# johnomotani/SharedMemSparseLU.jl

Measured on AMD Instinct MI355X. Metric: nnz(L+U)/s + achieved HBM GB/s, 3D Poisson 128³ numeric LU, 1/2/4/8 GPU, higher is better.
Workload: dtype f64

## Files before the change

sharedmemsparselu.jl_amd/csrc/plan.hpp:

```cpp
#pragma once
#include <algorithm>
#include <cstdint>
#include <string>
#include <vector>

namespace smlu {

struct Tune {
  int ob = 0;
  int64_t t128_min = 512;
  bool small_k = true;
  int64_t fullpiv_ns = -1;
  int64_t f22_gather_nu = 512;
  int64_t f22_gather_ch = 8;
  int64_t lside_min = 2048;
  int sweep_spin = 1 << 22;
  bool solve_steps = false;
  bool no_graph = false;
  bool debug_sync = false;
  bool no_repivot = false;
  int host_threads = 0;
};
Tune tune();


struct PlanOptions {
  int ordering = 0;
  int64_t grid[3] = {0, 0, 0};
  int relax = 1;
  int64_t leaf_size = 64;
  std::vector<int64_t> preorder;
};

struct Graph {
  int64_t n = 0;
  std::vector<int64_t> ptr;
  std::vector<int32_t> adj;
};

Graph build_sym_graph(int64_t n, const int64_t* colptr, const int32_t* rowval);
std::vector<int64_t> order_geometric_nd(int64_t nx, int64_t ny, int64_t nz, int64_t leaf);
std::vector<int64_t> order_graph_nd(const Graph& g, int64_t leaf);
std::vector<int64_t> order_amd(const Graph& g);
std::vector<int64_t> compute_order(int64_t n, const int64_t* colptr, const int32_t* rowval,
                                   const PlanOptions& opt, std::string& err);
std::vector<int64_t> zero_free_diagonal(int64_t n, const int64_t* colptr, const int32_t* rowval,
                                        const double* a);

struct Plan {
  int64_t n = 0, nnzA = 0;
  std::vector<int64_t> Acolptr;
  std::vector<int32_t> Arow;
  bool sym_pattern = false;

  std::vector<int64_t> q, qinv;
  std::vector<int64_t> p0, p0inv;
  bool given_order = false;
  bool matched = false;
  int perm_parity = 0;
  int pair_parity = -1;

  int64_t ntsup = 0;
  std::vector<int64_t> t_first;
  std::vector<int64_t> t_rowptr;
  std::vector<int32_t> t_rows;
  std::vector<int32_t> col2t;

  int64_t nsup = 0;
  std::vector<int64_t> s_first;
  std::vector<int64_t> s_parent;
  std::vector<int64_t> s_rowptr;
  std::vector<int32_t> s_rows;
  std::vector<int32_t> col2s;
  std::vector<int32_t> s_level;
  std::vector<int64_t> ch_ptr;
  std::vector<int32_t> ch_list;
  std::vector<int32_t> child_rank;
  std::vector<int32_t> relmap;
  int nlevels = 0;
  std::vector<int64_t> lev_ptr;
  std::vector<int32_t> lev_sup;

  std::vector<int64_t> Loff, Uoff;
  std::vector<int64_t> lev_foff;
  int64_t factor_size = 0;
  std::vector<int64_t> Foff;
  std::vector<int64_t> lev_soff, lev_ssize;
  int64_t scratch_size = 0;

  std::vector<int64_t> Adest;
  std::vector<int32_t> A_s, A_li, A_lj;
  std::vector<int64_t> Alev_ptr;
  std::vector<int32_t> Alev_ent;
  std::vector<int64_t> Arowptr;
  std::vector<int32_t> Arow_ent;

  double nnzL = 0, nnzU = 0;
  double upd = 0;
  double flops = 0;
  double stored = 0;
  int64_t front_max = 0, ns_max = 0, nu_max = 0;
  double analysis_ms = 0;
  double phase_ms[12] = {0};

  int nparts = 1;
  int64_t dob = 384;
// ... 51 lines not shown
```

sharedmemsparselu.jl_amd/csrc/schedule.hpp:

```cpp
#pragma once
#include <algorithm>
#include <cstdint>
#include <string>
#include <vector>

#include "device.hpp"
#include "plan.hpp"

namespace smlu {

constexpr int kSmallM = 128;
constexpr int kFullPivNs = 512;
constexpr int kNbFull = 32;
constexpr int kNbTile = 64;
constexpr int kSwapStride = 1 + 2 * 64;
constexpr int kOBDefault = 384;

enum Kind : int {
  K_EXTADD, K_FRONT_LDS, K_PANEL, K_TRSMU, K_TRSML,
  K_GEMM, K_FWD, K_BWD, K_FWDG, K_TRIF, K_BWDU, K_TRIB, K_GEMM22, K_LASWP, K_STEPTRSM, K_GEMMU,
  K_GEMMO, K_TRIINV, K_BWDU12C, K_VCOPY, K_FWDT, K_BWDT, K_SWEEPF, K_SWEEPB, K_UROWS, K_FWDP, K_NKIND
};
inline const char* const kKindName[] = {"assemble", "small", "panel",
                                  "trsm", "trsm", "gemm", "solve", "solve", "solve", "solve",
// ... 24 lines not shown
  int64_t so;
  int db;
  int64_t dof;
  int64_t bytes;
};

struct CommOp {
  int type = 0;
  std::vector<int32_t> peer;
  std::vector<int> sbase, rbase;
  std::vector<int64_t> soff, roff, sbytes, rbytes;
  int32_t root = -1;
  std::vector<int32_t> grp;
  int bbase = 4;
  int64_t bytes = 0;
  std::vector<HSeg> pack, unpack;
  int64_t pack0 = 0, unpack0 = 0;
  int at(int32_t p) {
    for (size_t i = 0; i < peer.size(); ++i)
      if (peer[i] == p) return (int)i;
    peer.push_back(p);
    sbase.push_back(4);
    rbase.push_back(5);
    soff.push_back(0);
    roff.push_back(0);
    sbytes.push_back(0);
    rbytes.push_back(0);
    return (int)peer.size() - 1;
  }
};

struct Operand {
  int buf = -1;
  int64_t off = 0;
  Operand operator+(int64_t d) const { return Operand{buf, off + d}; }
};
struct GemmRec {
  Operand A, B, C;
  int32_t m, n, k;
  int32_t lda, ldb, ldc;
  int32_t tiles_m = 0;
  int32_t gsid = -1;
  int64_t tile0 = 0;
  int32_t front = -1;
};

struct ScheduleInput {
  const Plan* plan = nullptr;
  const RankLayout* lay = nullptr;
  Tune tn;
  int rank = 0, nranks = 1;
  bool dominant = false;
  int pivmode = 0;
  bool cpair = false;
  bool use_mfma = true;
  int ob = kOBDefault;
};

struct Schedule {
  std::vector<SNode> hsn;
  std::vector<int32_t> node_front;
  int64_t nnodes = 0;
  std::vector<Launch> fac, fwd, bwd;
  std::vector<Launch> fwdm, bwdm;
  std::vector<size_t> fac_seg, fwd_seg, bwd_seg;
  std::vector<size_t> fwdm_seg, bwdm_seg;
  std::vector<int> fac_comm, fwd_comm, bwd_comm;
  std::vector<CommOp> comm;
  std::vector<int32_t> ilist;
  std::vector<XContrib> xt;
  std::vector<AEnt> ae;
  std::vector<XCol> xc;
  std::vector<FrontTile> ft;
  std::vector<int32_t> gptr, gent;
  std::vector<GemmRec> gt;
  std::vector<SwapTask> st_tasks;
  std::vector<URowTask> ur_tasks;
  std::vector<F22Gather> g22;
  std::vector<F22Child> g22ch;
  std::vector<int32_t> g22inv;
  int64_t f22_gather_fronts = 0;
  double f22_gather_entries = 0;
  int64_t side_launches = 0, side_rows = 0;
  double gemm_flops = 0, gemm22_flops = 0;
  double gemm_bytes = 0;
  int64_t gemm_launches = 0, gemm128_launches = 0;
  int64_t nlaunch = 0;
  int64_t max_list = 1;
  int64_t ssync_n = 0, ntick = 0;
  int64_t voff = 0;
  bool uses_tinv = false;
  int ob = kOBDefault;
  int64_t t128_min = 512;
  bool small_k = true;
  bool trsm_gemm = true;
  int err_code = 0;
};
constexpr int kSchedErrArg = -1, kSchedErrAlloc = -3, kSchedErrState = -6;

std::string build_schedule(const ScheduleInput& in, Schedule& out);
void rank_layout_of(const Plan& P, int rank, int nranks, RankLayout& Y);
void schedule_digest(const Schedule& S, const double bytes[5], std::vector<uint64_t>& out);

}
```

sharedmemsparselu.jl_amd/csrc/schedule_build.cpp:

```cpp
#include "schedule.hpp"

#include <limits>
#include <unordered_map>
#include <utility>

namespace smlu {
namespace {

const Operand kStore{0, 0}, kScratch{1, 0}, kBlockBuf{6, 0}, kTinv{7, 0};

GemmRec gemm_task(Operand A, Operand B, Operand C, int64_t m, int64_t n, int64_t k, int64_t lda, int64_t ldb,
                  int64_t ldc, int32_t gsid = -1) {
  GemmRec g;
  g.A = A; g.B = B; g.C = C;
  g.m = (int32_t)m; g.n = (int32_t)n; g.k = (int32_t)k;
  g.lda = (int32_t)lda; g.ldb = (int32_t)ldb; g.ldc = (int32_t)ldc;
  g.gsid = gsid;
  return g;
}
void update(std::vector<GemmRec>& cand, double& fl, Operand A, Operand B, Operand C, int64_t m, int64_t n, int64_t k,
            int64_t lda, int64_t ldb, int64_t ldc) {
  if (m <= 0 || n <= 0 || k <= 0) return;
  cand.push_back(gemm_task(A, B, C, m, n, k, lda, ldb, ldc));
  fl += 2.0 * (double)m * (double)n * (double)k;
// ... 21 lines not shown
  std::unordered_map<int64_t, int32_t> blkmap;
  std::vector<int64_t> fr_ptr;
  std::vector<int32_t> fr_ent;
  std::vector<int64_t> LP;
  std::vector<int32_t> LS;
  std::vector<std::vector<int32_t>> dfront;
  std::vector<char> dlevel;
  int64_t dist_slots = 0;
  int64_t spf = 0;
  int fuse_mode = 0;
  bool fuse_panel = false, fuse_inv = false, fuse_urows = false;
  std::vector<int64_t> bidx;
  std::vector<int32_t> col_cnt, col_pos;
  std::vector<std::vector<Launch>> bwd_levels;
  std::vector<char> f22g;
  int cur_level = 0;
  std::vector<size_t> lvl_end;

  Builder(const ScheduleInput& i, Schedule& s)
      : in(i), P(*i.plan), Y(*i.lay), S(s), rank(i.rank), nranks(i.nranks) {}

  static Launch launch(int kind, int step, size_t off) {
    Launch L;
    L.kind = kind;
    L.step = step;
    L.off = (int64_t)off;
    return L;
  }
  void fail(int code, const char* msg) {
    S.err_code = code;
    err = msg;
  }
  void add_comm(std::vector<Launch>& seq, std::vector<size_t>& seg, std::vector<int>& cm, CommOp&& op) {
    seg.push_back(seq.size());
    cm.push_back((int)S.comm.size());
    S.comm.push_back(std::move(op));
  }
  int32_t child_col(int64_t c, int64_t jc, int64_t* src) const {
    const int64_t nuc = P.nu(c);
    if (!P.dist(c)) {
      if (src && P.owner[c] == rank) *src = Y.Foff[c] + jc * nuc;
      return P.owner[c];
    }
    const int64_t b = P.npblk(c) + jc / P.dob;
    const int32_t o = P.blk_owner(c, b);
    if (src && o == rank) {
      const RankLayout::Blk& B = Y.blocks[blkmap.at((int64_t)c * 1048576 + b)];
      *src = B.foff + (P.ns(c) + jc - B.c0) * nuc;
    }
    return o;
  }
  int32_t node_of(int64_t s, int64_t b) const { return blknode[blkmap.at(s * 1048576 + b)]; }
  int32_t holder(int64_t c) const { return P.dist(c) ? P.blk_owner(c, P.npblk(c) - 1) : P.owner[c]; }
  bool gform(int64_t s) const { return S.trsm_gemm && S.hsn[s].nb == kNbTile; }
  int64_t slot_of(int64_t s, int64_t u) const { return dist_slots + bidx[s] * spf + u; }
  struct Step {
    int64_t kb, w, ostart, oend, R, M, slot;
  };
  Step geom(int64_t s, int64_t t) const {
    const SNode& r = S.hsn[s];
    Step g;
    g.M = (int64_t)r.ns + r.nu;
    g.kb = t * r.nb;
    g.w = std::min<int64_t>(r.nb, r.ns - g.kb);
    g.ostart = (g.kb / S.ob) * S.ob;
    g.oend = std::min<int64_t>(r.ns, g.ostart + S.ob);
    g.R = r.mode == 1 ? r.ns - g.kb : g.w;
    g.slot = slot_of(s, t % (S.ob / r.nb));
    return g;
  }
  void add_gemm_launch(std::vector<GemmRec>& cand, double fl, int step, int kind = K_GEMM, bool side = false) {
    if (cand.empty()) return;
    const bool count = kind != K_TRSML;
    int64_t t128 = 0;
    for (auto& g : cand) t128 += (int64_t)((g.m + 127) / 128) * ((g.n + 127) / 128);
    int tile = t128 >= S.t128_min && !(kind == K_TRSML && S.small_k) ? 128 : 64;
    if (tile == 128) tile = in.use_mfma ? kMfmaTile : 64;
    if (tile == 131 && step < 0) tile = 135;
    if (tile == 64 && S.small_k) {
      int kmax = 0;
      for (auto& g : cand) kmax = std::max(kmax, g.k);
      tile = kmax <= 64 ? 65 : in.use_mfma ? 66 : 64;
    }
    if (step < 0)
      std::stable_sort(cand.begin(), cand.end(), [](const GemmRec& a, const GemmRec& b) { return a.k > b.k; });
    Launch L = launch(step < 0 ? K_GEMM22 : kind, step, S.gt.size());
    if (step < 0 && !f22_gather(cand, tile, L)) return;
    L.aux = tile;
    int64_t tiles = 0;
    const int ts = tile >= 128 ? 128 : 64;
    for (GemmRec& g : cand) {
      if (count) S.gemm_bytes += 8.0 * ((double)g.m * g.k + (double)g.k * g.n + 2.0 * g.m * g.n);
      if (g.A.buf == kTinv.buf || g.B.buf == kTinv.buf) S.uses_tinv = true;
      g.tiles_m = (g.m + ts - 1) / ts;
      g.tile0 = tiles;
      tiles += (int64_t)g.tiles_m * ((g.n + ts - 1) / ts);
      S.gt.push_back(g);
    }
    L.cnt = (int64_t)cand.size();
    L.nwg = tiles;
    L.flops = fl;
    if (side) {
      L.side = true;
      L.grp = cur_level + 1;
      ++S.side_launches;
      if (kind == K_TRSML)
        for (const GemmRec& g : cand) S.side_rows += g.m;
    }
    S.fac.push_back(L);
    if (!count) return;
    S.gemm_flops += fl;
    ++S.gemm_launches;
    if (tile >= 128) ++S.gemm128_launches;
    if (step < 0) S.gemm22_flops += fl;
  }

  void choose_f22_gather(int l) {
    if (nranks > 1 || in.cpair || !in.use_mfma || in.tn.f22_gather_nu <= 0) return;
    int64_t t128 = 0;
    for (int64_t k = LP[l]; k < LP[l + 1]; ++k) {
      const SNode& r = S.hsn[LS[k]];
      if (r.mode != 0 && r.nu > 0 && r.ns > 0) t128 += (int64_t)((r.nu + 127) / 128) * ((r.nu + 127) / 128);
    }
    if (t128 < S.t128_min) return;
    for (int64_t k = LP[l]; k < LP[l + 1]; ++k) {
      const int64_t s = LS[k];
      const SNode& r = S.hsn[s];
      if (r.mode == 0 || r.ns <= 0 || r.nu < in.tn.f22_gather_nu) continue;
      int64_t nch = 0, numax = 0;
      for (int64_t e = P.ch_ptr[s]; e < P.ch_ptr[s + 1]; ++e) {
        nch += P.nu(P.ch_list[e]) > 0;
        numax = std::max(numax, P.nu(P.ch_list[e]));
      }
      if (nch <= in.tn.f22_gather_ch && numax <= 23170) f22g[s] = 1;
    }
  }
  bool f22_gather(const std::vector<GemmRec>& cand, int& tile, Launch& L) {
    bool any = false;
    for (const GemmRec& g : cand) any = any || (g.front >= 0 && f22g[g.front]);
    if (!any) return true;
    if (tile != 135) {
      fail(kSchedErrState, "internal: F22 gather chosen for a launch off the 128 MFMA tile");
      return false;
    }
    tile = kMfmaGatherTile;
    L.off2 = (int64_t)S.g22.size();
    std::vector<std::pair<int64_t, int64_t>> wr, rd;
    for (const GemmRec& g : cand) {
      wr.push_back({g.C.off, g.C.off + (int64_t)g.ldc * (g.n - 1) + g.m});
      if (g.front < 0 || !f22g[g.front]) {
        S.g22.push_back(F22Gather{0, -1});
        continue;
      }
      const int64_t s = g.front, ns = P.ns(s), nu = P.nu(s);
      F22Gather G{(int32_t)S.g22ch.size(), 0};
      for (int64_t e = P.ch_ptr[s]; e < P.ch_ptr[s + 1]; ++e) {
        const int64_t c = P.ch_list[e], nuc = P.nu(c);
        if (nuc <= 0) continue;
        const int32_t* rm = P.relmap.data() + S.hsn[c].rowptr;
        const int64_t inv0 = (int64_t)S.g22inv.size();
        S.g22inv.resize(inv0 + nu, -1);
        int32_t* inv = S.g22inv.data() + inv0;
        int64_t lo = nu, hi = -1, want = 0, have = 0;
        for (int64_t jc = 0; jc < nuc; ++jc) {
          const int64_t i = (int64_t)rm[jc] - ns;
          if (i < 0) continue;
          if (i >= nu) {
            fail(kSchedErrState, "internal: a child's row map leaves its parent front");
            return false;
          }
          inv[i] = (int32_t)jc;
          lo = std::min(lo, i);
          hi = std::max(hi, i);
          ++want;
        }
        for (int64_t i = 0; i < nu; ++i) have += inv[i] >= 0;
// ... 219 lines not shown
        S.xc.push_back(XCol{nodes[ri], tjf, base + cnt[tj], cnt[tj + 1] - cnt[tj],
                            (int32_t)((int64_t)S.ae.size() - a0), a0});
      }
  }
  void assembly(int l, const RecvAt& recv_at) {
    Launch L = launch(K_EXTADD, 0, S.xc.size());
    for (int64_t k = LP[l]; k < LP[l + 1]; ++k) {
      const int64_t s = LS[k];
      if (S.hsn[s].mode != 0) front_columns(s, {{0, P.M(s)}}, {(int32_t)s}, recv_at);
    }
    for (const int32_t t : dfront[l]) {
      std::vector<std::pair<int64_t, int64_t>> ranges;
      std::vector<int32_t> nodes;
      for (size_t i = 0; i < Y.blocks.size(); ++i)
        if (Y.blocks[i].s == t) {
          ranges.push_back({Y.blocks[i].c0, Y.blocks[i].c1});
          nodes.push_back(blknode[i]);
        }
      front_columns(t, ranges, nodes, recv_at);
    }
    L.cnt = (int64_t)S.xc.size() - L.off;
    if (L.cnt > 0) S.fac.push_back(L);
  }

  void small_fronts(int l) {
    const int64_t cls[6] = {16, 32, 48, 64, 96, kSmallM};
    for (int c = 0; c < 6; ++c) {
      Launch L = launch(K_FRONT_LDS, 0, S.ilist.size());
      int64_t Mmax = 0;
      for (int64_t k = LP[l]; k < LP[l + 1]; ++k) {
        int64_t s = LS[k];
        if (S.hsn[s].mode != 0) continue;
        int64_t M = P.M(s);
        if (M > cls[c] || (c > 0 && M <= cls[c - 1])) continue;
        S.ilist.push_back((int32_t)s);
        S.ilist.push_back((int32_t)S.ae.size());
        S.ilist.push_back((int32_t)(fr_ptr[s + 1] - fr_ptr[s]));
        for (int64_t e = fr_ptr[s]; e < fr_ptr[s + 1]; ++e) {
          const int32_t id = fr_ent[e];
          S.ae.push_back(AEnt{id, (int32_t)((P.A_lj[id] << 16) | P.A_li[id])});
        }
        Mmax = std::max(Mmax, M);
      }
      L.cnt = ((int64_t)S.ilist.size() - L.off) / 3;
      L.aux = Mmax;
      L.aux2 = l + 1;
      if (L.cnt > 0) S.fac.push_back(L);
    }
    std::vector<std::pair<int64_t, int64_t>> wr, rd;
    for (int64_t k = LP[l]; k < LP[l + 1]; ++k) {
      const int64_t s = LS[k];
      if (S.hsn[s].mode != 0) continue;
      const int64_t nu = P.nu(s);
      if (nu > 0 && S.hsn[s].Foff >= 0) wr.push_back({S.hsn[s].Foff, S.hsn[s].Foff + nu * nu});
      for (int64_t e = P.ch_ptr[s]; e < P.ch_ptr[s + 1]; ++e) {
        const int64_t c = P.ch_list[e], nuc = P.nu(c);
        if (nuc > 0 && S.hsn[c].Foff >= 0) rd.push_back({S.hsn[c].Foff, S.hsn[c].Foff + nuc * nuc});
      }
    }
    std::sort(wr.begin(), wr.end());
    for (size_t i = 1; i < wr.size(); ++i)
      if (wr[i].first < wr[i - 1].second) {
        fail(kSchedErrState, "internal: overlapping F22 blocks in one level");
        return;
      }
    for (const auto& r : rd) {
      auto it = std::upper_bound(wr.begin(), wr.end(), std::make_pair(r.second, (int64_t)-1));
      if (it != wr.begin() && std::prev(it)->second > r.first) {
        fail(kSchedErrState, "internal: a level's F22 block overlaps a child's F22 it reads");
        return;
      }
    }
  }

  void blocked_fronts(int l) {
    std::vector<int64_t> big;
    int64_t maxsteps = 0;
    for (int64_t k = LP[l]; k < LP[l + 1]; ++k) {
      int64_t s = LS[k];
      const SNode& r = S.hsn[s];
      if (r.mode == 0) continue;
      bidx[s] = (int64_t)big.size();
      big.push_back(s);
      maxsteps = std::max<int64_t>(maxsteps, (r.ns + r.nb - 1) / r.nb);
    }
    S.max_list = std::max<int64_t>(S.max_list, dist_slots + (int64_t)big.size() * spf);
    for (int64_t t = 0; t < maxsteps; ++t) {
      std::vector<int64_t> act;
      for (auto s : big) {
        const SNode& r = S.hsn[s];
        if (t * r.nb < r.ns) act.push_back(s);
      }
      if (act.empty()) continue;
      step_panels(t, act);
      if (!err.empty()) return;
      step_solves(t, act);
      std::vector<int64_t> fin_all;
      for (auto s : act) {
        const Step g = geom(s, t);
        if (g.kb + g.w == g.oend) fin_all.push_back(s);
      }
      if (!fin_all.empty()) outer_block_end(t, fin_all);
    }
    std::vector<GemmRec> cand;
    double fl = 0;
    for (auto s : big) {
      const SNode& r = S.hsn[s];
      const size_t had = cand.size();
      update(cand, fl, kStore + r.Loff + r.ns, kStore + r.Uoff, kScratch + r.Foff, r.nu, r.nu, r.ns,
             (int64_t)r.ns + r.nu, r.ns, r.nu);
      if (cand.size() > had) cand.back().front = (int32_t)s;
    }
    add_gemm_launch(cand, fl, -1);
  }
  int pclass(int64_t s, int64_t t) const {
    const SNode& r = S.hsn[s];
    if (r.nb > 32) return 0;
    const int64_t R = r.mode == 1 ? r.ns - t * r.nb : std::min<int64_t>(r.nb, r.ns - t * r.nb);
    return R <= 64 ? 1 : R <= 128 ? 2 : R <= 256 ? 3 : R <= 512 ? 4 : 5;
  }
  void step_panels(int64_t t, std::vector<int64_t>& act) {
    std::stable_sort(act.begin(), act.end(), [&](int64_t a, int64_t b) { return pclass(a, t) < pclass(b, t); });
    size_t pos = 0;
    for (int c = 0; c < 6 && pos < act.size(); ++c) {
      Launch L = launch(K_PANEL, (int)t, S.ilist.size());
      int64_t rmax = 1, wmax = 1, cnt = 0;
      while (pos < act.size() && pclass(act[pos], t) == c) {
        const Step g = geom(act[pos], t);
        rmax = std::max(rmax, g.R);
        wmax = std::max<int64_t>(wmax, S.hsn[act[pos]].nb);
        S.ilist.push_back((int32_t)act[pos]);
        S.ilist.push_back((int32_t)g.slot);
        ++pos;
        ++cnt;
      }
      L.cnt = cnt;
      L.aux = 0;
      L.nwg = rmax;
      L.aux2 = wmax;
      L.cnt2 = c == 0 ? fuse_mode : 0;
      if (L.cnt > 0) S.fac.push_back(L);
    }
    if (pos != act.size()) fail(kSchedErrArg, "internal: panel classes");
  }
  void step_solves(int64_t t, const std::vector<int64_t>& act) {
    Launch L;
    L.kind = K_TRIINV;
    L.step = (int)t;
    L.off = (int64_t)S.ilist.size();
    for (auto s : act) {
      if (!gform(s) || fuse_inv) continue;
      S.ilist.push_back((int32_t)s);
      S.ilist.push_back((int32_t)geom(s, t).slot);
    }
    L.cnt = ((int64_t)S.ilist.size() - L.off) / 2;
    if (L.cnt > 0) S.fac.push_back(L);
    L = launch(K_LASWP, (int)t, S.st_tasks.size());
    int64_t wg = 0;
    for (auto s : act) {
      const Step g = geom(s, t);
      const int64_t ncol = g.oend - g.ostart - g.w;
      if (ncol <= 0 || (fuse_panel && gform(s))) continue;
      S.st_tasks.push_back(SwapTask{(int32_t)s, (int32_t)g.kb, 1, (int32_t)g.slot, (int32_t)g.ostart,
                                    (int32_t)g.oend, (int32_t)g.kb, (int32_t)(g.kb + g.w), wg});
      wg += (ncol + 63) / 64;
    }
// ... 66 lines not shown
           S.hsn[s].mode == 2 && g.M - g.oend >= in.tn.lside_min;
  }
  void lside_check() {
    if (S.side_launches == 0) return;
    struct Pos {
      int64_t row, col, oend, M;
    };
    auto where = [&](const GemmRec& g, const Operand& X, Pos& p) {
      if (g.front < 0 || X.buf != kStore.buf) return false;
      const SNode& r = S.hsn[g.front];
      p.M = (int64_t)r.ns + r.nu;
      const int64_t rel = X.off - r.Loff;
      if (rel < 0 || rel >= p.M * r.ns) return false;
      p.col = rel / p.M;
      p.row = rel % p.M;
      p.oend = std::min<int64_t>(r.ns, (p.col / S.ob + 1) * S.ob);
      return true;
    };
    std::vector<char> pend(P.nsup, 0);
    std::vector<int32_t> plist;
    size_t lv = 0, plevel = 0;
    for (size_t i = 0; i < S.fac.size(); ++i) {
      while (lv < lvl_end.size() && lvl_end[lv] <= i) ++lv;
      const Launch& L = S.fac[i];
      const bool step_gemm = L.kind == K_TRSML || L.kind == K_GEMM;
      if (L.side) {
        if (!step_gemm || L.grp != (int)lv + 1) return fail(kSchedErrState, "internal: a side launch of another kind or level");
        for (int64_t j = L.off; j < L.off + L.cnt; ++j) {
          const GemmRec& g = S.gt[j];
          Pos c{}, a{};
          bool ok = where(g, g.C, c) && S.hsn[g.front].mode == 2 && c.row >= c.oend && c.row + g.m <= c.M &&
                    c.col + g.n <= c.oend;
          if (ok && L.kind == K_GEMM) ok = where(g, g.A, a) && a.row == c.row && a.oend == c.oend;
          if (!ok) return fail(kSchedErrState, "internal: a side task reaches above its outer block's end");
          if (!pend[g.front]) {
            pend[g.front] = 1;
            plist.push_back(g.front);
          }
        }
        plevel = lv;
        continue;
      }
      if (plist.empty()) continue;
      if (fac_joins_side(L.kind)) {
        for (const int32_t f : plist) pend[f] = 0;
        plist.clear();
        continue;
      }
      if (lv != plevel) return fail(kSchedErrState, "internal: side launches not joined before the next level");
      if (!step_gemm) continue;
      for (int64_t j = L.off; j < L.off + L.cnt; ++j) {
        const GemmRec& g = S.gt[j];
        Pos c{};
        if (g.front < 0 || !pend[g.front]) continue;
        if (!where(g, g.C, c) || c.row + g.m > c.oend)
          return fail(kSchedErrState, "internal: a main-stream task writes rows a pending side launch owns");
      }
    }
  }
  void outer_block_end(int64_t t, const std::vector<int64_t>& fin_all) {
    Launch L = launch(K_LASWP, (int)t, S.st_tasks.size());
    int64_t wg = 0;
    for (auto s : fin_all) {
      const SNode& r = S.hsn[s];
      const Step g = geom(s, t);
      const int64_t ncol = g.M - (g.oend - g.ostart);
      if (ncol <= 0) continue;
      S.st_tasks.push_back(SwapTask{(int32_t)s, (int32_t)g.ostart, (int32_t)((g.oend - g.ostart + r.nb - 1) / r.nb),
                                    (int32_t)slot_of(s, (g.ostart % S.ob) / r.nb), 0, (int32_t)g.M,
                                    (int32_t)g.ostart, (int32_t)g.oend, wg});
      wg += (ncol + 63) / 64;
    }
    L.cnt = (int64_t)S.st_tasks.size() - L.off;
    L.nwg = wg;
    if (wg > 0) S.fac.push_back(L);
    std::vector<URows> items;
    std::vector<GemmRec> c1;
    double fl1 = 0;
    for (auto s : fin_all) {
      const SNode& r = S.hsn[s];
      const Step g = geom(s, t);
      if (g.oend == g.M) continue;
      items.push_back(URows{s, g.ostart, g.oend, g.oend, r.ns, true});
      rank_update(s, g.oend, g.M, g.oend, r.ns, false, g.ostart, g.oend, c1, fl1);
      rank_update(s, g.oend, r.ns, g.oend, g.oend, true, g.ostart, g.oend, c1, fl1);
    }
    urows(t, items);
    add_gemm_launch(c1, fl1, (int)t, K_GEMMO);
  }
  struct URows {
    int64_t s, ob0, ob1, c0, c1;
    bool u12;
  };
  void urows(int64_t t, const std::vector<URows>& all_items) {
    std::vector<URows> items;
    Launch L = launch(K_UROWS, (int)t, S.ur_tasks.size());
    for (auto& it : all_items) {
      const SNode& r = S.hsn[it.s];
      if (!(fuse_urows && gform(it.s))) {
        items.push_back(it);
        continue;
      }
      const int64_t M = (int64_t)r.ns + r.nu;
      const int32_t slot0 = (int32_t)slot_of(it.s, (it.ob0 % S.ob) / r.nb);
      for (int64_t c = it.c0; c < it.c1; c += kUrowsCols)
        S.ur_tasks.push_back(URowTask{(int32_t)it.s, (int32_t)it.ob0, (int32_t)it.ob1, slot0, (int32_t)M,
                                      (int32_t)std::min<int64_t>(kUrowsCols, it.c1 - c), r.Loff + c * M});
      if (it.u12)
        for (int64_t c = 0; c < r.nu; c += kUrowsCols)
          S.ur_tasks.push_back(URowTask{(int32_t)it.s, (int32_t)it.ob0, (int32_t)it.ob1, slot0, r.ns,
                                        (int32_t)std::min<int64_t>(kUrowsCols, r.nu - c), r.Uoff + c * r.ns});
    }
    L.cnt = (int64_t)S.ur_tasks.size() - L.off;
    if (L.cnt > 0) S.fac.push_back(L);
    int64_t nsub = 0;
    for (auto& it : items) nsub = std::max<int64_t>(nsub, (it.ob1 - it.ob0 + S.hsn[it.s].nb - 1) / S.hsn[it.s].nb);
    for (int64_t u = 0; u < nsub; ++u) {
      L = Launch();
      L.kind = K_TRSMU;
      L.step = (int)t;
      L.aux = 1;
      L.off = (int64_t)S.ft.size();
      int64_t wg = 0, cnt = 0;
      std::vector<GemmRec> cand, ctri;
      double fl = 0;
      for (auto& it : items) {
        const int64_t s = it.s;
        const SNode& r = S.hsn[s];
        const int64_t M = (int64_t)r.ns + r.nu;
        const int64_t kbu = it.ob0 + u * r.nb;
        if (kbu >= it.ob1) continue;
        const int64_t wu = std::min<int64_t>(r.nb, it.ob1 - kbu);
        const int64_t n1 = it.c1 - it.c0;
        const Operand F = kStore + r.Loff, U = kStore + r.Uoff;
        const bool u12 = it.u12 && r.nu > 0;
        if (gform(s)) {
          const Operand Ti = tinv_at(slot_of(s, (kbu % S.ob) / r.nb), false);
          if (n1 > 0) ctri.push_back(gemm_task(Ti, F + it.c0 * M + kbu, F + it.c0 * M + kbu, wu, n1, wu, 64, M, M));
          if (u12) ctri.push_back(gemm_task(Ti, U + kbu, U + kbu, wu, r.nu, wu, 64, r.ns, r.ns));
        } else {
          S.ft.push_back(FrontTile{(int32_t)s, (int32_t)kbu, wg});
          wg += (M - it.c0 + 255) / 256;
          ++cnt;
        }
        const int64_t m = it.ob1 - kbu - wu;
        update(cand, fl, F + kbu * M + kbu + wu, F + it.c0 * M + kbu, F + it.c0 * M + kbu + wu, m, n1, wu, M, M, M);
        if (u12) update(cand, fl, F + kbu * M + kbu + wu, U + kbu, U + kbu + wu, m, r.nu, wu, M, r.ns, r.ns);
      }
      L.cnt = cnt;
      L.nwg = wg;
      if (wg > 0) S.fac.push_back(L);
      add_gemm_launch(ctri, 0.0, (int)t, K_TRSML);
      add_gemm_launch(cand, fl, (int)t, K_GEMMU);
    }
  }
  void rank_update(int64_t s, int64_t r0, int64_t r1, int64_t c0, int64_t c1, bool u12, int64_t k0, int64_t k1,
                   std::vector<GemmRec>& cand, double& fl) {
    const SNode& r = S.hsn[s];
    const int64_t M = (int64_t)r.ns + r.nu;
    const Operand F = kStore + r.Loff, U = kStore + r.Uoff;
    update(cand, fl, F + k0 * M + r0, F + c0 * M + k0, F + c0 * M + r0, r1 - r0, c1 - c0, k1 - k0, M, M, M);
    const int64_t ru1 = std::min<int64_t>(r1, r.ns);
    if (u12) update(cand, fl, F + k0 * M + r0, U + k0, U + r0, ru1 - r0, r.nu, k1 - k0, M, r.ns, r.ns);
  }

  void shared_front(int32_t t) {
    const int64_t np = P.npblk(t);
    std::vector<size_t> mine;
    for (size_t i = 0; i < Y.blocks.size(); ++i)
      if (Y.blocks[i].s == t) mine.push_back(i);
    std::vector<Launch> pending;
    for (int64_t b = 0; b < np; ++b) {
      const bool own = P.blk_owner(t, b) == rank;
      const int32_t bn = own ? node_of(t, b) : -1;
      if (own) shared_block_factor(t, b, bn);
      shared_block_bcast(t, b, bn);
      for (auto& q : pending) S.fac.push_back(q);
      pending.clear();
      shared_block_apply(t, b, bn, mine, pending);
    }
    for (auto& q : pending) S.fac.push_back(q);
  }
  void shared_block_factor(int32_t t, int64_t b, int32_t bn) {
    const int64_t M = P.M(t), ob = P.blk_c0(t, b), oe = P.blk_c1(t, b);
    const Operand Lb = kStore + S.hsn[bn].Loff;
    for (int64_t kb = ob; kb < oe; kb += 64) {
      const int64_t wk = std::min<int64_t>(64, oe - kb);
      const int step = (int)(kb / 64);
      const int32_t u = (int32_t)((kb - ob) / 64);
      Launch Q = launch(K_PANEL, step, S.ilist.size());
      S.ilist.push_back(bn);
      S.ilist.push_back(u);
      Q.cnt = 1;
      Q.nwg = wk;
      Q.aux2 = 64;
      S.fac.push_back(Q);
      Q = launch(K_TRIINV, step, S.ilist.size());
      S.ilist.push_back(bn);
      S.ilist.push_back(u);
      Q.cnt = 1;
      S.fac.push_back(Q);
      if (oe - ob - wk > 0) {
        Q = launch(K_LASWP, step, S.st_tasks.size());
        S.st_tasks.push_back(SwapTask{bn, (int32_t)kb, 1, u, (int32_t)ob, (int32_t)oe, (int32_t)kb,
                                      (int32_t)(kb + wk), 0});
        Q.cnt = 1;
        Q.nwg = (oe - ob - wk + 63) / 64;
        S.fac.push_back(Q);
      }
      std::vector<GemmRec> tri, cand;
      double fl = 0;
      if (oe - kb - wk > 0) {
        const Operand X = Lb + (kb + wk) * M + kb;
        tri.push_back(gemm_task(tinv_at(u, false), X, X, wk, oe - kb - wk, wk, 64, M, M));
      }
      if (M - kb - wk > 0) {
        const Operand X = Lb + kb * M + kb + wk;
        tri.push_back(gemm_task(X, tinv_at(u, true), X, M - kb - wk, wk, wk, M, 64, M, bn));
      }
      add_gemm_launch(tri, 0.0, step, K_TRSML);
      update(cand, fl, Lb + kb * M + kb + wk, Lb + (kb + wk) * M + kb, Lb + (kb + wk) * M + kb + wk, M - kb - wk,
             oe - kb - wk, wk, M, M, M);
      add_gemm_launch(cand, fl, step);
    }
  }
  void shared_block_bcast(int32_t t, int64_t b, int32_t bn) {
    const SNode& fr = S.hsn[t];
    const int64_t M = P.M(t), ob = P.blk_c0(t, b), oe = P.blk_c1(t, b), w = oe - ob, nsub = (w + 63) / 64;
    const int64_t lbytes = 8 * (M - ob) * w, tbytes = 8 * nsub * 8192;
    const int64_t swbytes = 4 * nsub * kSwapStride, rpbytes = 4 * w;
    CommOp op;
    op.type = 1;
    op.root = P.blk_owner(t, b);
    op.grp = P.group[t];
    op.bytes = lbytes + tbytes + swbytes + rpbytes;
    if (op.root == rank) {
      op.bbase = 4;
      for (int64_t c = ob; c < oe; ++c)
        op.pack.push_back(HSeg{0, 8 * (S.hsn[bn].Loff + c * M + ob), 4, 8 * (c - ob) * (M - ob), 8 * (M - ob)});
      op.pack.push_back(HSeg{7, 0, 4, lbytes, tbytes});
      op.pack.push_back(HSeg{8, 0, 4, lbytes + tbytes, swbytes});
      op.pack.push_back(HSeg{9, 4 * (fr.first + ob), 4, lbytes + tbytes + swbytes, rpbytes});
    } else {
      op.bbase = 6;
      op.unpack.push_back(HSeg{6, lbytes + tbytes, 8, 0, swbytes});
      op.unpack.push_back(HSeg{6, lbytes + tbytes + swbytes, 9, 4 * (fr.first + ob), rpbytes});
// ... 377 lines not shown
        }
      }
      if (!op.peer.empty()) add_comm(S.bwd, S.bwd_seg, S.bwd_comm, std::move(op));
    }
    int32_t prev = -1;
    bool first = true;
    for (int64_t ub = np; ub < nbk; ++ub) {
      const int32_t o = P.blk_owner(t, ub);
      if (prev >= 0) vhop(S.bwd, S.bwd_seg, S.bwd_comm, prev, o, tv, ns);
      if (rank == o) {
        Launch L;
        L.kind = K_BWDU12C;
        L.node = node_of(t, ub);
        L.aux = P.blk_c0(t, ub);
        L.aux2 = P.blk_c1(t, ub);
        L.cnt = first ? 1 : 0;
        S.bwd.push_back(L);
      }
      prev = o;
      first = false;
    }
    if (first) {
      prev = P.blk_owner(t, np - 1);
      if (rank == prev) {
        Launch L;
        L.kind = K_VCOPY;
        L.node = t;
        S.bwd.push_back(L);
      }
    }
    for (int64_t b = np - 1; b >= 0; --b) {
      const int32_t o = P.blk_owner(t, b);
      const int64_t ob = P.blk_c0(t, b), oe = P.blk_c1(t, b);
      vhop(S.bwd, S.bwd_seg, S.bwd_comm, prev, o, tv, oe);
      if (rank == o) tri_steps(true, node_of(t, b), ob, oe, S.bwd);
      prev = o;
    }
  }

  void expand(const Launch& Sw, bool upper, std::vector<Launch>& out) {
    std::vector<int32_t> fr;
    for (int64_t i = Sw.off; i < Sw.off + Sw.cnt; ++i) fr.push_back(S.ft[i].s);
    int64_t nb = 0;
    for (auto s : fr) nb = std::max<int64_t>(nb, (S.hsn[s].ns + 63) / 64);
    for (int64_t t = 0; t < nb; ++t) {
      Launch F;
      F.kind = upper ? K_TRIB : K_TRIF;
      F.grp = Sw.grp;
      F.step = (int)t;
      F.off = (int64_t)S.ft.size();
      int64_t w = 0, cnt = 0;
      for (auto s : fr) {
        const SNode& r = S.hsn[s];
        const int64_t nbs = (r.ns + 63) / 64;
        if (t >= nbs) continue;
        S.ft.push_back(FrontTile{s, 0, w});
        w += tri_wg(upper, (int64_t)r.ns + r.nu, r.ns, (upper ? nbs - 1 - t : t) * 64);
        ++cnt;
      }
      F.cnt = cnt;
      F.nwg = w;
      out.push_back(F);
    }
  }
  void expand_all(const std::vector<Launch>& seq, const std::vector<size_t>& seg, bool upper,
                  std::vector<Launch>& out, std::vector<size_t>& oseg) {
    std::vector<size_t> at(seq.size() + 1);
    for (size_t i = 0; i < seq.size(); ++i) {
      at[i] = out.size();
      if (seq[i].kind == (upper ? K_SWEEPB : K_SWEEPF)) expand(seq[i], upper, out);
      else out.push_back(seq[i]);
    }
    at[seq.size()] = out.size();
    oseg.clear();
    for (size_t k : seg) oseg.push_back(at[std::min(k, seq.size())]);
  }

  std::string run() {
    S = Schedule();
    S.ob = in.tn.ob > 0 ? in.tn.ob : in.ob;
    S.t128_min = in.tn.t128_min;
    S.small_k = in.tn.small_k;
    S.trsm_gemm = in.use_mfma;
    nodes();
    group_entries();
    levels();
    f22g.assign(P.nsup, 0);
    for (int l = 0; l < P.nlevels && err.empty(); ++l) {
      cur_level = l;
      choose_f22_gather(l);
      assembly(l, f22_exchange(l));
      small_fronts(l);
      if (err.empty()) blocked_fronts(l);
      if (!err.empty()) break;
      for (const int32_t t : dfront[l]) shared_front(t);
      lvl_end.push_back(S.fac.size());
    }
    if (err.empty()) lside_check();
    for (int l = 0; l < P.nlevels && err.empty(); ++l) {
      solve_level(l);
      for (const int32_t t : dfront[l]) shared_forward(t);
    }
    if (!err.empty()) return err;
    backward();
    S.nlaunch = (int64_t)S.fac.size();
    expand_all(S.fwd, S.fwd_seg, false, S.fwdm, S.fwdm_seg);
    expand_all(S.bwd, S.bwd_seg, true, S.bwdm, S.bwdm_seg);
    if (nranks > 1) S.max_list = std::max<int64_t>(S.max_list, dist_slots);
    return err;
  }
};

}

std::string build_schedule(const ScheduleInput& in, Schedule& out) { return Builder(in, out).run(); }

void rank_layout_of(const Plan& P, int rank, int nranks, RankLayout& Y) {
  if (nranks > 1) {
    rank_layout(P, rank, Y);
    return;
  }
  Y = RankLayout();
  Y.Loff = P.Loff;
  Y.Uoff = P.Uoff;
  Y.Foff = P.Foff;
  Y.recv_off.assign(P.nsup, -1);
  Y.recv_size.assign(P.nsup, 0);
  Y.store_size = P.factor_size;
  Y.scratch_size = P.scratch_size;
}

}
```

sharedmemsparselu.jl_amd/csrc/smlu.cpp:

```cpp
#include "handle.hpp"

namespace smlu {
thread_local std::string g_last_error;
}

static int check_device(smlu_handle* h) {
  int cnt = 0;
  hipError_t e = hipGetDeviceCount(&cnt);
  if (e != hipSuccess || cnt <= 0)
    return fail(h, SMLU_ERR_NODEVICE, "no HIP device visible (libsmlu has no CPU fallback)");
  if (h->opts.device < 0 || h->opts.device >= cnt)
    return fail(h, SMLU_ERR_NODEVICE, "opts.device out of range");
  hipDeviceProp_t prop;
  if (hipGetDeviceProperties(&prop, h->opts.device) != hipSuccess)
    return fail(h, SMLU_ERR_NODEVICE, "hipGetDeviceProperties failed");
  if (std::strncmp(prop.gcnArchName, "gfx950", 6) != 0)
    return fail(h, SMLU_ERR_NODEVICE, std::string("device is ") + prop.gcnArchName + ", libsmlu is built for gfx950 only");
  h->device = h->opts.device;
  return SMLU_OK;
}

std::vector<int64_t> diagonal_match(int64_t n, const int64_t* colptr, const int64_t* rowval,
                                    const double* a, int64_t base) {
  bool need = false;
// ... 194 lines not shown
  if (k == "repivot_info") return (double)h->repivot_info;
  if (k == "repivot_growth") return h->repivot_growth;
  if (k == "repivot_node_mode" || k == "repivot_node_ns" || k == "repivot_node_nu") {
    if (h->repivot_node < 0) return -1;
    const SNode& r = h->repivot_sn;
    return k == "repivot_node_mode" ? r.mode : k == "repivot_node_ns" ? r.ns : r.nu;
  }
  if (k == "pivot_tol") return h->opts.pivot_tol;
  if (k == "diag_pivot_tol") return h->plan.given_order ? 0.0 : h->opts.diag_pivot_tol;
  if (k == "sweep_timeouts") {
    return (double)h->sweep_timeouts;
  }
  if (k == "solve_passes") {
    return (double)h->solve_passes;
  }
  if (k == "solve_trans_passes") {
    return (double)h->trans_passes;
  }
  if (k == "rcond_solves") return (double)h->rcond_solves;
  if (k == "rcond_solves_fwd") return (double)h->rcond_solves_fwd;
  if (k == "rcond_solves_adj") return (double)h->rcond_solves_adj;
  if (k == "rcond_iters") return (double)h->rcond_iters;
  if (k == "logabsdet_evals") return (double)h->logabsdet_evals;
  if (k == "gmres_iters") return (double)h->gmres_iters;
  if (k == "gmres_cycles") return (double)h->gmres_cycles;
  if (k == "gmres_solves") return (double)h->gmres_solves;
  if (k == "gmres_ms_last") return h->gmres_ms;
  if (k == "sweep_status") {
    int32_t v = 0;
    if (h->sstatus.p && hipMemcpy(&v, h->sstatus.p, sizeof v, hipMemcpyDeviceToHost) != hipSuccess) return -1;
    return v;
  }
  if (k == "solve_sweeps") {
    int64_t c = 0;
    for (const Launch& L : h->sch.fwd) c += L.kind == K_SWEEPF;
    for (const Launch& L : h->sch.bwd) c += L.kind == K_SWEEPB;
    return (double)c;
  }
  if (k.rfind("launches_", 0) == 0) {
    const std::string v = k.substr(9);
    double c = 0;
    for (const Launch& L : h->sch.fac) {
      const bool gemm = L.kind == K_GEMM || L.kind == K_GEMMU || L.kind == K_GEMMO || L.kind == K_GEMM22;
      const bool trsm = L.kind == K_TRSML;
      const bool mfma = L.aux == 131 || L.aux == 135 || L.aux == 143;
      if (v == "mfma128" && gemm && mfma) ++c;
      else if (v == "mfma128_gather" && gemm && L.aux == 143) ++c;
      else if (v == "mfma128_trsm" && trsm && mfma) ++c;
      else if (v == "k64" && gemm && L.aux == 65) ++c;
      else if (v == "k64_trsm" && trsm && L.aux == 65) ++c;
      else if (v == "valu64" && gemm && L.aux == 64) ++c;
      else if (v == "mfma64" && gemm && L.aux == 66) ++c;
      else if (v == "valu64_trsm" && trsm && L.aux == 64) ++c;
      else if (v == "tri_inv" && L.kind == K_TRIINV) ++c;
      else if (v == "panel_tall" && L.kind == K_PANEL && L.nwg > 512) ++c;
    }
    return c;
  }
  if (k.rfind("fronts_mode", 0) == 0) {
    const int m = std::atoi(k.c_str() + 11);
    double c = 0;
    for (const SNode& r : h->sch.hsn) c += r.mode == m ? 1 : 0;
    return c;
  }
  if (k == "pattern_dropped") return (double)h->pattern_dropped;
  if (k == "given_pattern") return h->given_pattern ? 1.0 : 0.0;
  if (k == "status_copy_retries") return (double)h->status_copy_retries;
  if (k == "bad_info_count") return (double)h->bad_info_count;
  if (k == "bad_info_node") return (double)h->bad_info_node;
  if (k == "bad_info_word") return (double)h->bad_info_word;
  if (k == "refine_steps") return (double)h->refine_steps;
  if (k == "refine_residual") return h->refine_resid;
  if (k == "refine_berr") return h->refine_berr;
  if (k == "refine_batch_residuals") return (double)h->refine_batch_residuals;
  if (k == "gemm_flops") return h->sch.gemm_flops;
  if (k == "gemm22_flops") return h->sch.gemm22_flops;
  if (k == "gemm_launches") return (double)h->sch.gemm_launches;
  if (k == "gemm_bytes") return h->sch.gemm_bytes;
  if (k == "f22_gather_fronts") return (double)h->sch.f22_gather_fronts;
  if (k == "f22_gather_entries") return h->sch.f22_gather_entries;
  if (k == "gemm128_launches") return (double)h->sch.gemm128_launches;
  if (k == "side_launches") return (double)h->sch.side_launches;
  if (k == "side_rows") return (double)h->sch.side_rows;
  if (k == "vendor_calls") return 0.0;
  if (k.rfind("ms_", 0) == 0) {
    std::string name = k.substr(3);
    double t = 0;
    bool found = false;
    for (int i = 0; i < K_NKIND; ++i)
      if (name == kKindName[i]) { t += h->kind_ms[i]; found = true; }
    return found ? t : std::numeric_limits<double>::quiet_NaN();
  }
  return plan_stat(h->plan, k);
}

int smlu_plan_create(int64_t n, const int64_t* colptr, const int64_t* rowval, const smlu_opts* opts,
                     smlu_plan** out) {
  if (!out || !colptr || n <= 0) return fail(nullptr, SMLU_ERR_ARG, "invalid arguments");
  smlu_opts o;
  if (opts) o = *opts;
  else smlu_default_opts(&o);
  if (!valid_opts(&o)) return fail(nullptr, SMLU_ERR_ARG, "index_base must be 0 or 1");
  std::unique_ptr<smlu_plan> p(new smlu_plan());
  std::string e = p->plan.build(n, colptr, rowval, o.index_base, plan_opts(o));
  if (!e.empty()) return fail(nullptr, SMLU_ERR_ARG, e);
  *out = p.release();
  return SMLU_OK;
}

double smlu_plan_stat(const smlu_plan* plan, const char* key) {
  if (!plan || !key) return std::numeric_limits<double>::quiet_NaN();
  return plan_stat(plan->plan, key);
}

int smlu_plan_pattern(const smlu_plan* pl, int64_t* q, int64_t* Lcolptr, int64_t* Lrowval) {
  if (!pl) return SMLU_ERR_ARG;
  const Plan& P = pl->plan;
  if (q) for (int64_t i = 0; i < P.n; ++i) q[i] = P.q[i];
  if (Lcolptr || Lrowval) {
    int64_t o = 0;
    if (Lcolptr) Lcolptr[0] = 0;
    for (int64_t j = 0; j < P.n; ++j) {
      int64_t t = P.col2t[j], last = P.t_first[t + 1] - 1;
      if (Lrowval) {
        for (int64_t i = j; i <= last; ++i) Lrowval[o++] = i;
        for (int64_t e = P.t_rowptr[t]; e < P.t_rowptr[t + 1]; ++e) Lrowval[o++] = P.t_rows[e];
      } else {
        o += last - j + 1 + P.t_rowptr[t + 1] - P.t_rowptr[t];
      }
      if (Lcolptr) Lcolptr[j + 1] = o;
    }
  }
  return SMLU_OK;
}

int smlu_plan_supernodes(const smlu_plan* pl, int64_t* first, int64_t* parent, int64_t* level) {
  if (!pl) return SMLU_ERR_ARG;
  const Plan& P = pl->plan;
  for (int64_t s = 0; s <= P.nsup; ++s)
    if (first) first[s] = P.s_first[s];
  for (int64_t s = 0; s < P.nsup; ++s) {
    if (parent) parent[s] = P.s_parent[s];
    if (level) level[s] = P.s_level[s];
  }
  return SMLU_OK;
}

static void fronts_of(const Plan& P, int64_t* first, int64_t* parent, int64_t* rowptr, int64_t* rows,
                      int64_t* p0) {
  for (int64_t s = 0; s <= P.nsup; ++s) {
    if (first) first[s] = P.s_first[s];
    if (rowptr) rowptr[s] = P.s_rowptr[s];
  }
  for (int64_t s = 0; s < P.nsup; ++s)
    if (parent) parent[s] = P.s_parent[s];
  if (rows)
    for (int64_t e = 0; e < P.s_rowptr[P.nsup]; ++e) rows[e] = P.s_rows[e];
  if (p0)
    for (int64_t i = 0; i < P.n; ++i) p0[i] = P.p0[i];
}

int smlu_plan_fronts(const smlu_plan* pl, int64_t* rowptr, int64_t* rows, int64_t* p0) {
  if (!pl) return SMLU_ERR_ARG;
  fronts_of(pl->plan, nullptr, nullptr, rowptr, rows, p0);
  return SMLU_OK;
}
// ... 16 lines not shown
```

sharedmemsparselu.jl_amd/csrc/tune.cpp:

```cpp
#include <algorithm>
#include <cstdlib>

#include "plan.hpp"

namespace smlu {

Tune tune() {
  Tune v;
  {
    if (const char* e = std::getenv("SMLU_OB")) v.ob = std::max(64, (std::atoi(e) / 64) * 64);
    if (const char* e = std::getenv("SMLU_T128MIN")) v.t128_min = std::atoll(e);
    if (const char* e = std::getenv("SMLU_SMALLK")) v.small_k = std::atoi(e) != 0;
    if (const char* e = std::getenv("SMLU_FULLPIV_NS")) v.fullpiv_ns = std::atoll(e);
    if (const char* e = std::getenv("SMLU_F22_GATHER_NU")) v.f22_gather_nu = std::atoll(e);
    if (const char* e = std::getenv("SMLU_F22_GATHER_CH")) v.f22_gather_ch = std::atoll(e);
    if (const char* e = std::getenv("SMLU_LSIDE_MIN")) v.lside_min = std::max<long long>(0, std::atoll(e));
    if (const char* e = std::getenv("SMLU_SWEEP_SPIN")) v.sweep_spin = std::atoi(e);
    if (const char* e = std::getenv("SMLU_SOLVE_STEPS")) v.solve_steps = std::atoi(e) == 1;
    v.no_graph = std::getenv("SMLU_NO_GRAPH") != nullptr;
    v.debug_sync = std::getenv("SMLU_DEBUG_SYNC") != nullptr;
    v.no_repivot = std::getenv("SMLU_NO_REPIVOT") != nullptr;
    if (const char* e = std::getenv("OMP_NUM_THREADS")) v.host_threads = std::atoi(e);
  }
  return v;
}

}
```

Before: 7.044 billion.

## Defer trailing updates in large fronts using binary-span recursive rank updates

For large single-GPU fronts (ns >= 1024), the per-step outer trailing update is restructured so that updates accumulate over several panel blocks, using a binary-counter span pattern. This yields fewer, larger-k GEMMs instead of many rank-ob updates, which should raise GEMM efficiency and cut how often the trailing matrix is read and written. GEMMO candidates are now sorted by k, and a schedule validator checks that every block has received all its trailing updates before its panel or the F22 update runs. The cost is a more complex dependency pattern plus extra host-side checking during schedule build.

```diff
diff --git a/sharedmemsparselu.jl_amd/csrc/plan.hpp b/sharedmemsparselu.jl_amd/csrc/plan.hpp
--- a/sharedmemsparselu.jl_amd/csrc/plan.hpp
+++ b/sharedmemsparselu.jl_amd/csrc/plan.hpp
@@ -14,6 +14,8 @@
   int64_t f22_gather_nu = 512;
   int64_t f22_gather_ch = 8;
   int64_t lside_min = 2048;
+  int trail_span = 2;
+  int64_t trail_ns = 1024;
   int sweep_spin = 1 << 22;
   bool solve_steps = false;
   bool no_graph = false;
@@ -22,6 +24,7 @@
   int host_threads = 0;
 };
 Tune tune();
+constexpr int64_t kTrailNsMin = 1024, kTrailNsTest = 64;
 
 
 struct PlanOptions {
diff --git a/sharedmemsparselu.jl_amd/csrc/schedule.hpp b/sharedmemsparselu.jl_amd/csrc/schedule.hpp
--- a/sharedmemsparselu.jl_amd/csrc/schedule.hpp
+++ b/sharedmemsparselu.jl_amd/csrc/schedule.hpp
@@ -130,6 +130,7 @@
   int64_t f22_gather_fronts = 0;
   double f22_gather_entries = 0;
   int64_t side_launches = 0, side_rows = 0;
+  int64_t trail_span = 1, trail_fronts = 0, gemmo_kmax = 0;
   double gemm_flops = 0, gemm22_flops = 0;
   double gemm_bytes = 0;
   int64_t gemm_launches = 0, gemm128_launches = 0;
diff --git a/sharedmemsparselu.jl_amd/csrc/schedule_build.cpp b/sharedmemsparselu.jl_amd/csrc/schedule_build.cpp
--- a/sharedmemsparselu.jl_amd/csrc/schedule_build.cpp
+++ b/sharedmemsparselu.jl_amd/csrc/schedule_build.cpp
@@ -127,7 +127,7 @@
       for (auto& g : cand) kmax = std::max(kmax, g.k);
       tile = kmax <= 64 ? 65 : in.use_mfma ? 66 : 64;
     }
-    if (step < 0)
+    if (step < 0 || kind == K_GEMMO)
       std::stable_sort(cand.begin(), cand.end(), [](const GemmRec& a, const GemmRec& b) { return a.k > b.k; });
     Launch L = launch(step < 0 ? K_GEMM22 : kind, step, S.gt.size());
     if (step < 0 && !f22_gather(cand, tile, L)) return;
@@ -137,6 +137,7 @@
     for (GemmRec& g : cand) {
       if (count) S.gemm_bytes += 8.0 * ((double)g.m * g.k + (double)g.k * g.n + 2.0 * g.m * g.n);
       if (g.A.buf == kTinv.buf || g.B.buf == kTinv.buf) S.uses_tinv = true;
+      if (kind == K_GEMMO) S.gemmo_kmax = std::max<int64_t>(S.gemmo_kmax, g.k);
       g.tiles_m = (g.m + ts - 1) / ts;
       g.tile0 = tiles;
       tiles += (int64_t)g.tiles_m * ((g.n + ts - 1) / ts);
@@ -522,6 +523,7 @@
       if (r.mode == 0) continue;
       bidx[s] = (int64_t)big.size();
       big.push_back(s);
+      S.trail_fronts += trail(s);
       maxsteps = std::max<int64_t>(maxsteps, (r.ns + r.nb - 1) / r.nb);
     }
     S.max_list = std::max<int64_t>(S.max_list, dist_slots + (int64_t)big.size() * spf);
@@ -754,8 +756,18 @@
       const Step g = geom(s, t);
       if (g.oend == g.M) continue;
       items.push_back(URows{s, g.ostart, g.oend, g.oend, r.ns, true});
-      rank_update(s, g.oend, g.M, g.oend, r.ns, false, g.ostart, g.oend, c1, fl1);
-      rank_update(s, g.oend, r.ns, g.oend, g.oend, true, g.ostart, g.oend, c1, fl1);
+      int64_t k0 = g.ostart, e = r.ns;
+      if (trail(s) && g.oend < r.ns) {
+        const int64_t j = g.oend / S.ob, span = in.tn.trail_span, b = j & -j;
+        if (span > 0 && j % span == 0) {
+          k0 = (j - span) * S.ob;
+        } else {
+          k0 = (j - b) * S.ob;
+          e = std::min<int64_t>(r.ns, (j + b) * S.ob);
+        }
+      }
+      rank_update(s, g.oend, g.M, g.oend, e, false, k0, g.oend, c1, fl1);
+      rank_update(s, g.oend, e, e, r.ns, true, k0, g.oend, c1, fl1);
     }
     urows(t, items);
     add_gemm_launch(c1, fl1, (int)t, K_GEMMO);
@@ -831,9 +843,90 @@
     const SNode& r = S.hsn[s];
     const int64_t M = (int64_t)r.ns + r.nu;
     const Operand F = kStore + r.Loff, U = kStore + r.Uoff;
+    const size_t had = cand.size();
     update(cand, fl, F + k0 * M + r0, F + c0 * M + k0, F + c0 * M + r0, r1 - r0, c1 - c0, k1 - k0, M, M, M);
     const int64_t ru1 = std::min<int64_t>(r1, r.ns);
     if (u12) update(cand, fl, F + k0 * M + r0, U + k0, U + r0, ru1 - r0, r.nu, k1 - k0, M, r.ns, r.ns);
+    for (size_t i = had; i < cand.size(); ++i) cand[i].front = (int32_t)s;
+  }
+
+  bool trail(int64_t s) const {
+    const SNode& r = S.hsn[s];
+    return nranks == 1 && in.tn.trail_span != 1 && in.dominant && in.pivmode == 0 && !in.cpair && gform(s) &&
+           r.mode == 2 && r.ns >= in.tn.trail_ns;
+  }
+  void trail_check() {
+    if (S.trail_fronts == 0) return;
+    struct Fr {
+      int64_t nB = 0;
+      std::vector<int32_t> done;
+    };
+    std::unordered_map<int32_t, Fr> fr;
+    auto front = [&](int32_t s) -> Fr& {
+      Fr& f = fr[s];
+      if (f.done.empty()) {
+        f.nB = (S.hsn[s].ns + S.ob - 1) / S.ob;
+        f.done.assign((size_t)((f.nB + 1) * (f.nB + 1)), 0);
+      }
+      return f;
+    };
+    const char* const bad = "internal: a trailing update out of tree order";
+    for (const Launch& L : S.fac) {
+      if (L.kind == K_GEMMO) {
+        for (int64_t i = L.off; i < L.off + L.cnt; ++i) {
+          const GemmRec& g = S.gt[i];
+          if (g.front < 0 || !trail(g.front)) continue;
+          const SNode& r = S.hsn[g.front];
+          Fr& f = front(g.front);
+          const int64_t ns = r.ns, M = ns + r.nu, ob = S.ob;
+          const int64_t a = g.A.off - r.Loff, c = g.C.off - r.Loff, cu = g.C.off - r.Uoff;
+          const bool u12 = !(c >= 0 && c < M * ns);
+          if (g.A.buf != kStore.buf || g.B.buf != kStore.buf || g.C.buf != kStore.buf || a < 0 || a >= M * ns ||
+              g.lda != M || (u12 && (r.nu == 0 || cu < 0 || cu >= ns * r.nu)))
+            return fail(kSchedErrState, bad);
+          const int64_t k0 = a / M, k1 = k0 + g.k, r0 = a % M, r1 = r0 + g.m;
+          const int64_t c0 = u12 ? ns : c / M, c1 = u12 ? M : c0 + g.n;
+          const int64_t ld = u12 ? ns : M, crow = u12 ? cu % ns : c % M, ccol = u12 ? cu / ns : 0;
+          const bool ok = g.ldc == ld && g.ldb == ld && crow == r0 && ccol == 0 && (!u12 || g.n == r.nu) &&
+                          g.B.off == (u12 ? r.Uoff : r.Loff + c0 * M) + k0 && k0 % ob == 0 && k1 % ob == 0 &&
+                          k1 == geom(g.front, L.step).oend && k1 < ns && r0 % ob == 0 && r0 >= k1 && r0 < ns &&
+                          (r1 == M || (r1 <= ns && (r1 % ob == 0 || r1 == ns))) && (!u12 || r1 <= ns) &&
+                          (u12 || (c0 % ob == 0 && c0 >= k1 && c1 <= ns && (c1 % ob == 0 || c1 == ns)));
+          if (!ok) return fail(kSchedErrState, bad);
+          const int64_t br1 = r1 > ns ? f.nB + 1 : (r1 + ob - 1) / ob;
+          const int64_t bc0 = u12 ? f.nB : c0 / ob, bc1 = u12 ? f.nB + 1 : (c1 + ob - 1) / ob;
+          for (int64_t br = r0 / ob; br < br1; ++br)
+            for (int64_t bc = bc0; bc < bc1; ++bc) {
+              int32_t& d = f.done[(size_t)(br * (f.nB + 1) + bc)];
+              if (d != k0 / ob || k1 / ob > std::min(br, bc)) return fail(kSchedErrState, bad);
+              d = (int32_t)(k1 / ob);
+            }
+        }
+      } else if (L.kind == K_PANEL) {
+        for (int64_t i = L.off; i < L.off + 2 * L.cnt; i += 2) {
+          const int32_t s = S.ilist[i];
+          if (!trail(s)) continue;
+          const Step g = geom(s, L.step);
+          if (g.kb != g.ostart) continue;
+          const Fr& f = front(s);
+          const int64_t j = g.ostart / S.ob;
+          for (int64_t q = j; q < f.nB + (S.hsn[s].nu > 0); ++q)
+            if (f.done[(size_t)(q * (f.nB + 1) + j)] != j || f.done[(size_t)(j * (f.nB + 1) + q)] != j)
+              return fail(kSchedErrState, "internal: an outer block starts before its trailing updates are complete");
+        }
+      } else if (L.kind == K_GEMM22) {
+        for (int64_t i = L.off; i < L.off + L.cnt; ++i) {
+          const int32_t s = S.gt[i].front;
+          if (s < 0 || !trail(s)) continue;
+          const Fr& f = front(s);
+          for (int64_t br = 0; br <= f.nB; ++br)
+            for (int64_t bc = 0; bc <= f.nB; ++bc)
+              if (br + bc < 2 * f.nB && f.done[(size_t)(br * (f.nB + 1) + bc)] != std::min(br, bc))
+                return fail(kSchedErrState, "internal: an F22 update before the front's trailing updates are complete");
+          fr.erase(s);
+        }
+      }
+    }
   }
 
   void shared_front(int32_t t) {
@@ -1377,6 +1470,7 @@
     S.t128_min = in.tn.t128_min;
     S.small_k = in.tn.small_k;
     S.trsm_gemm = in.use_mfma;
+    S.trail_span = in.tn.trail_span;
     nodes();
     group_entries();
     levels();
@@ -1392,6 +1486,7 @@
       lvl_end.push_back(S.fac.size());
     }
     if (err.empty()) lside_check();
+    if (err.empty()) trail_check();
     for (int l = 0; l < P.nlevels && err.empty(); ++l) {
       solve_level(l);
       for (const int32_t t : dfront[l]) shared_forward(t);
diff --git a/sharedmemsparselu.jl_amd/csrc/smlu.cpp b/sharedmemsparselu.jl_amd/csrc/smlu.cpp
--- a/sharedmemsparselu.jl_amd/csrc/smlu.cpp
+++ b/sharedmemsparselu.jl_amd/csrc/smlu.cpp
@@ -300,6 +300,9 @@
   if (k == "gemm128_launches") return (double)h->sch.gemm128_launches;
   if (k == "side_launches") return (double)h->sch.side_launches;
   if (k == "side_rows") return (double)h->sch.side_rows;
+  if (k == "trail_span") return (double)h->sch.trail_span;
+  if (k == "trail_fronts") return (double)h->sch.trail_fronts;
+  if (k == "gemmo_kmax") return (double)h->sch.gemmo_kmax;
   if (k == "vendor_calls") return 0.0;
   if (k.rfind("ms_", 0) == 0) {
     std::string name = k.substr(3);
diff --git a/sharedmemsparselu.jl_amd/csrc/tune.cpp b/sharedmemsparselu.jl_amd/csrc/tune.cpp
--- a/sharedmemsparselu.jl_amd/csrc/tune.cpp
+++ b/sharedmemsparselu.jl_amd/csrc/tune.cpp
@@ -15,6 +15,15 @@
     if (const char* e = std::getenv("SMLU_F22_GATHER_NU")) v.f22_gather_nu = std::atoll(e);
     if (const char* e = std::getenv("SMLU_F22_GATHER_CH")) v.f22_gather_ch = std::atoll(e);
     if (const char* e = std::getenv("SMLU_LSIDE_MIN")) v.lside_min = std::max<long long>(0, std::atoll(e));
+    if (const char* e = std::getenv("SMLU_TRAIL_SPAN")) {
+      const int s = std::max(0, std::atoi(e));
+      v.trail_span = s;
+      while (v.trail_span & (v.trail_span - 1)) v.trail_span &= v.trail_span - 1;
+    }
+    if (const char* e = std::getenv("SMLU_TRAIL_NS")) {
+      const long long r = std::atoll(e);
+      v.trail_ns = r == kTrailNsTest ? r : std::max<long long>(kTrailNsMin, r);
+    }
     if (const char* e = std::getenv("SMLU_SWEEP_SPIN")) v.sweep_spin = std::atoi(e);
     if (const char* e = std::getenv("SMLU_SOLVE_STEPS")) v.solve_steps = std::atoi(e) == 1;
     v.no_graph = std::getenv("SMLU_NO_GRAPH") != nullptr;
```

After: 7.124 billion, median of 6. +1.1%, better.
